# joey156/MECH5845M-WBC-for-Legged-Manipulator

Measured on AMD Instinct MI355X. Metric: wbc_qp_solves_per_sec, higher is better.
Workload: dtype f64

## Files before the change

mech5845m-wbc-for-legged-manipulator_amd/csrc/wbc_k_sim3p.hip:

```cpp
#include "wbc_packed.h"

namespace wbc {

#ifdef WBC_ABLATE
#define PSTOP(k, val) do { if (A.dbg_stop == 100 + (k)) { if (valid) { A.out.qdot[(size_t)b * NV + s] = (val); if (s == 0) A.out.status[b] = 0; } return; } } while (0)
#else
#define PSTOP(k, val) do { } while (0)
#endif
#ifdef SIM3P_NO_LAYOUT_HINTS
#define RARE(c) (c)
#else
#define RARE(c) __builtin_expect(!!(c), 0)
#endif
#define COLD_MARK() asm volatile("; WBC_COLD")
#ifndef SIM3P_WAVES
#define SIM3P_WAVES 2
#endif
template <bool WARM, bool TRUNK = false, bool QCON = false, bool ROT = false, bool TP = false, bool FIXD = false>
#ifdef SIM3P_NUM_VGPR
__attribute__((amdgpu_waves_per_eu(SIM3P_NUM_VGPR, SIM3P_NUM_VGPR)))
#endif
__global__ void __launch_bounds__(64, SIM3P_WAVES) wbc_tick_sim3p_kernel(const KernelArgs A, const DevModel* __restrict__ models,
                                                               const WbcConfig* __restrict__ cfgs, const DevPlan* __restrict__ plans,
                                                               const WbcTaskParams* __restrict__ tps, const WoGeom wg) {
#ifdef SIM3P_NUM_VGPR
  extern __shared__ double dyn_lds_[];
  union SUU { SmemP P; Smem G; };
  SUU& SU = *reinterpret_cast<SUU*>(dyn_lds_);
#else
  __shared__ union { SmemP P; Smem G; } SU;
#endif
  static_assert(sizeof(Smem) <= 20480 && sizeof(SmemP) <= 20480, "8 waves per CU");
  SmemP& SP = SU.P;
  const int lane = threadIdx.x, r = lane >> 4, s = lane & 15, rbase = lane & 48;
  PInst& I = SP.I[r];
  PVec& V = SP.V[r];
  const int grp = (int)blockIdx.x;
  const int pos = 4 * grp + r;
  const bool valid = pos < A.B;
  const int b = valid ? wo_instance(A.worder, wg, A.B, grp, r, pos) : A.B - 1;
  int mid = 0;
  if (A.in.model_id) { mid = A.in.model_id[b]; mid = mid < 0 ? 0 : (mid >= A.n_models ? A.n_models - 1 : mid); }
  const DevModel& M = models[mid];
  const WbcConfig& cfg = cfgs[mid];
  const DevPlan& P = plans[mid];
  const double dt = A.dt, inv_dt = 1.0 / A.dt;
  const WbcTaskParams* tpr = nullptr;
  bool tpbad = false;
  if (TP) {
    tpbad = tp_row_bad16(tps + b, s, rbase);
    tpr = tpbad ? reinterpret_cast<const WbcTaskParams*>(&cfg.ee_W[0][0]) : tps + b;
  }

  {
    const double* qg = A.in.q + (size_t)b * NQ;
    const double q0 = qg[s], q1 = (16 + s < NQ) ? qg[16 + s] : 0.0;
    double ex = 0.0;
    if (s < 3) ex = A.in.ee_target ? A.in.ee_target[(size_t)b * 15 + 12 + s] : 0.0;
    else if (s < 6) ex = A.in.prev_ee_target ? A.in.prev_ee_target[(size_t)b * 15 + 12 + (s - 3)] : 0.0;
    else if (s < 10) ex = A.in.trunk_box_center ? A.in.trunk_box_center[(size_t)b * 4 + (s - 6)] : 0.0;
    V.in[s] = q0;
    if (16 + s < 28) V.in[16 + s] = q1;
    if (s < 10) V.in[28 + s] = ex;
    V.cl[s] = 0.0; V.cl[16 + s] = 0.0;
    if (TRUNK) {
      static_assert(offsetof(PVec, tv) - offsetof(PVec, yv) == 16 * sizeof(double), "yv [14..15] runs on into tv");
      double* const tin = V.yv + 14;
      const double t0 = pk_trunk_input(A.in, b, s), t1 = (s < 2) ? pk_trunk_input(A.in, b, 16 + s) : 0.0;
      const double tw = (s < 13) ? (TP ? (&tpr->trunk_W[0])[s] : (&cfg.trunk_W[0])[s]) : 0.0;
      tin[s] = t0;
      if (s < 2) tin[16 + s] = t1;
      if (s < 13) V.xv[2 + s] = tw;
    }
    if (WARM && s < 2) {
      const unsigned long long w = (A.ws_in && valid) ? A.ws_in[2 * (size_t)b + s] : 0ull;
      V.in[38 + s] = __longlong_as_double((long long)w);
    }
    if (A.in.ee_ref_rot) {
      if (s < 9) { V.dv[s] = A.in.ee_ref_rot[(size_t)b * 45 + 36 + s]; V.yv[s] = A.in.ee_prev_rot[(size_t)b * 45 + 36 + s]; }
    }
  }
  double at6[6] = {0, 0, 0, 0, 0, 0};
  if (TRUNK) {
    WSYNC();
    const double* const qv = V.in;
    const double* tw = V.xv + 2;
    double Rt_[9], vel[6];
    pk_trunk_target_vel(qv, V.yv + 14, tw, I.M2, inv_dt, s, Rt_, vel);
    const double trunk_w = tw[6];
    double at[6] = {0, 0, 0, 0, 0, 0};
    {
      const int c = s < 3 ? s : (s < 6 ? s - 3 : 0);
      const double col[3] = {Rt_[c], Rt_[3 + c], Rt_[6 + c]};
      const double pr[3] = {qv[0], qv[1], qv[2]};
      double lin[3] = {col[0], col[1], col[2]}, ang[3] = {0, 0, 0};
      if (s >= 3) { ang[0] = col[0]; ang[1] = col[1]; ang[2] = col[2]; cross3(pr, ang, lin); }
#pragma unroll
      for (int rr = 0; rr < 3; ++rr) {
        at[rr] = (s < 6) ? (tw[rr] * lin[rr]) * trunk_w : 0.0;
        at[3 + rr] = (s < 6) ? (tw[3 + rr] * ang[rr]) * trunk_w : 0.0;
      }
    }
    double* const At2 = I.M1;
    WSYNC();
    if (s < 6) {
#pragma unroll
      for (int rr = 0; rr < 6; rr += 2) sts2(At2 + s * 6 + rr, at[rr], at[rr + 1]);
    }
    WSYNC();
#pragma unroll
    for (int rr = 0; rr < 6; ++rr) at6[rr] = at[rr];
    if (s < 6) {
      double vs = vel[0];
#pragma unroll
      for (int i = 1; i < 6; ++i) vs = (s == i) ? vel[i] : vs;
      V.pad_[s] = vs * trunk_w;
    }
    if (s < 6) {
      double gs = 0.0;
#pragma unroll
      for (int rr = 0; rr < 6; ++rr) gs = fma(-at[rr], vel[rr] * trunk_w, gs);
#pragma unroll
      for (int k = 0; k < 6; ++k) {
        const double2a t0 = lds2(At2 + k * 6), t1 = lds2(At2 + k * 6 + 2), t2 = lds2(At2 + k * 6 + 4);
        I.Cq[s * 6 + k] = fma(at[0], t0.x, fma(at[1], t0.y, fma(at[2], t1.x, fma(at[3], t1.y, fma(at[4], t2.x, at[5] * t2.y)))));
      }
      I.Cq[36 + s] = gs;
    }
    WSYNC();
    __builtin_amdgcn_sched_barrier(0);
  }
  const int nv = FIXD ? SIM3P_FIXD_NV : M.nv, nq = FIXD ? SIM3P_FIXD_NQ : M.nq, n = FIXD ? SIM3P_FIXD_N : P.n_red, nelim = FIXD ? SIM3P_FIXD_NELIM : P.nelim,
            nl = 3 * nelim, p_keep = FIXD ? SIM3P_FIXD_PKEEP : P.p_keep, p = p_keep + nl;
  const unsigned fl = P.flags;
  const bool c_con_trunk = fl & 2u;
  const int c_task_joint = (fl >> 4) & 7u;
  const bool has_grip = (P.task_ee_mask >> 4) & 1u;
  const DevPlan::PkCol cv = P.pk_var[s], cg = P.pk_leg[s];
  DevPlan::PkJoint fkn = P.pk_fk[0][s];
  const int scq0 = P.pk_scq[(2 + s) & 31], scq1 = P.pk_scq[(18 + s) & 31];
  const int dof0 = cv.dof, dof1 = cg.dof;
  const int c0_joint = cv.joint, c0_lin = cv.lin, c0_ang = cv.ang, c1_joint = cg.joint, c1_lin = cg.lin, c1_ang = cg.ang;
  const int dq0 = cv.dq_idx, dq1 = cg.dq_idx;
  const double dlo0 = cv.d_lo, dhi0 = cv.d_hi, dvm0 = cv.d_vm, dlo1 = cg.d_lo, dhi1 = cg.d_hi, dvm1 = cg.d_vm;
  const double dcoef = cfg.damper_coef, dqi = cfg.damper_qi, dqs = cfg.damper_qs;
  const int gj = M.frame_joint[WBC_FR_EE0 + 4];
  const double gp0 = M.frame_p[WBC_FR_EE0 + 4][0], gp1 = M.frame_p[WBC_FR_EE0 + 4][1], gp2 = M.frame_p[WBC_FR_EE0 + 4][2];
  const unsigned gsup = P.redsup[WBC_FR_EE0 + 4];
  const double ee_w = TPW(ee_w[4]);
  double eW[6], eG[3];
#pragma unroll
  for (int i = 0; i < 6; ++i) eW[i] = TPW(ee_W[4][i]);
#pragma unroll
  for (int i = 0; i < 3; ++i) eG[i] = TPW(ee_gain[4][i]);
  const double joint_w = TPW(joint_w), tb_z = cfg.trunk_box_z_frac, tb_a = cfg.trunk_box_ang, tb_s = cfg.trunk_box_scale;
  WSYNC();
  const double* const qv = V.in;
  PSTOP(6, qv[s] + dlo0 + dlo1 + eW[0] + (double)(fkn.joint + scq0 + scq1));
  double* const oMi = I.M1;
  double* const sc = I.M2 + PV * PLD - 48;
  pk_fk_seed(oMi, sc, qv, scq0, scq1, s);
  WSYNC();
  PSTOP(7, oMi[12 + s] + sc[4 + s]);
  pk_fk_sweep<ROT>(oMi, sc, qv, M, P.pk_fk, fkn, s);
  PSTOP(1, oMi[12 * 4 + (s & 7)]);
  double lin0[3] = {0, 0, 0}, ang0[3] = {0, 0, 0}, lin1[3] = {0, 0, 0};
  if (s < n) pk_jac_col(oMi, c0_joint, c0_lin, c0_ang, lin0, ang0);
  if (s < nl) { double a1[3]; pk_jac_col(oMi, c1_joint, c1_lin, c1_ang, lin1, a1); }
  double Rtr[9], ptr[3], pfe[3];
  {
    const double* Pr = oMi + 12 * M.frame_joint[WBC_FR_TRUNK];
#pragma unroll
    for (int c = 0; c < 3; ++c)
#pragma unroll
      for (int rr = 0; rr < 3; ++rr) Rtr[3 * rr + c] = Pr[3 * c + rr];
    ptr[0] = Pr[9]; ptr[1] = Pr[10]; ptr[2] = Pr[11];
    const double* Pg = oMi + 12 * gj;
#pragma unroll
    for (int rr = 0; rr < 3; ++rr) pfe[rr] = Pg[9 + rr] + Pg[rr] * gp0 + Pg[3 + rr] * gp1 + Pg[6 + rr] * gp2;
  }
  WSYNC();

  double* const At = I.M2;
  double* const Kb = I.M2 + 16 * 6;
  double* const Bb = I.M2 + 16 * 6 + 48;
  double g = 0.0;
  double a[6] = {0, 0, 0, 0, 0, 0};
  double bt[6] = {0, 0, 0, 0, 0, 0};
  if (has_grip) {
    const bool sup = (s < n) && ((gsup >> s) & 1u);
    double wxp[3];
    cross3(ang0, pfe, wxp);
#pragma unroll
    for (int rr = 0; rr < 3; ++rr) {
      a[rr] = sup ? eW[rr] * ((lin0[rr] + wxp[rr]) * ee_w) : 0.0;
      a[3 + rr] = sup ? eW[3 + rr] * (ang0[rr] * ee_w) : 0.0;
    }
    const double* xt = V.in + 28;
    const double* xp = V.in + 31;
#pragma unroll
    for (int i = 0; i < 3; ++i) {
      const double br = ((xt[i] - xp[i]) * inv_dt + eG[i] * ((xt[i] - pfe[i]) * inv_dt)) * ee_w;
      g = fma(-a[i], br, g);
      bt[i] = br;
    }
    if (A.in.ee_ref_rot) {
      const double* Rs = V.dv;
      const double* Rp = V.yv;
      double D[9];
#pragma unroll
      for (int i = 0; i < 9; ++i) D[i] = (Rs[i] - Rp[i]) * inv_dt;
      const double w3 = D[6] * Rs[3] + D[7] * Rs[4] + D[8] * Rs[5];
      const double w4 = D[0] * Rs[6] + D[1] * Rs[7] + D[2] * Rs[8];
      const double w5 = D[3] * Rs[0] + D[4] * Rs[1] + D[5] * Rs[2];
      g = fma(-a[3], w3 * ee_w, g); g = fma(-a[4], w4 * ee_w, g); g = fma(-a[5], w5 * ee_w, g);
      bt[3] = w3 * ee_w; bt[4] = w4 * ee_w; bt[5] = w5 * ee_w;
    }
  }
  if (TRUNK && s < 6) g += I.Cq[36 + s];
#pragma unroll
  for (int rr = 0; rr < 6; rr += 2) sts2(At + s * 6 + rr, a[rr], a[rr + 1]);
  if (!QCON) {
    if (s < nl) { Kb[4 * s] = lin1[0]; Kb[4 * s + 1] = lin1[1]; Kb[4 * s + 2] = lin1[2]; }
    if (s < 6) { Bb[4 * s] = lin0[0]; Bb[4 * s + 1] = lin0[1]; Bb[4 * s + 2] = lin0[2]; }
  }
  const double dpost = (1.0 / nv) * joint_w;
  double g1 = 0.0;
  double bp0 = 0.0, bp1 = 0.0;
  {
    const bool prev0 = (c_task_joint == WBC_JOINT_PREV) || (c_task_joint >= WBC_JOINT_MANI && !((P.post_zero >> dof0) & 1u));
    const bool prev1 = (c_task_joint == WBC_JOINT_PREV) || (c_task_joint >= WBC_JOINT_MANI && !((P.post_zero >> dof1) & 1u));
    double u0 = (prev0 && s < n) ? qv[dof0 < 6 ? dof0 : dof0 + 1] : 0.0;
    double u1 = (prev1 && s < nl) ? qv[dof1 < 6 ? dof1 : dof1 + 1] : 0.0;
    if (QCON && A.in.posture_u) {
      u0 = (s < n) ? A.in.posture_u[(size_t)b * NV + dof0] : 0.0;
      u1 = (s < nl) ? A.in.posture_u[(size_t)b * NV + dof1] : 0.0;
    }
    if (s < n) g = fma(-dpost, (1.0 / nv) * u0 * joint_w, g);
    if (s < nl) g1 = -dpost * ((1.0 / nv) * u1 * joint_w);
    bp0 = (s < n) ? (1.0 / nv) * u0 * joint_w : 0.0;
    bp1 = (s < nl) ? (1.0 / nv) * u1 * joint_w : 0.0;
  }
  if (s >= n) g = 0.0;
  if (RARE(A.post_static && P.post_pert)) {
    COLD_MARK();
    WSYNC();
    if (((P.post_pert >> s) & 1u)) V.in[s] = (qv[s] + 0.0002) - (0.0002 * 2);
    if (16 + s < NQ && ((P.post_pert >> (16 + s)) & 1u)) V.in[16 + s] = (qv[16 + s] + 0.0002) - (0.0002 * 2);
  }
  WSYNC();
  if (s < 6) {
    double v = bt[0];
#pragma unroll
    for (int i = 1; i < 6; ++i) v = (s == i) ? bt[i] : v;
    V.in[28 + s] = v;
  }
  double h[PV];
  {
#pragma unroll
    for (int k = 0; k < PV; ++k) {
      const double2a t0 = lds2(At + k * 6), t1 = lds2(At + k * 6 + 2), t2 = lds2(At + k * 6 + 4);
      h[k] = fma(a[0], t0.x, fma(a[1], t0.y, fma(a[2], t1.x, fma(a[3], t1.y, fma(a[4], t2.x, a[5] * t2.y)))));
    }
#pragma unroll
    for (int k = 0; k < PV; ++k) if (k == s) h[k] += (s < n) ? dpost * dpost : 1.0;
    if (TRUNK && s < 6) {
#pragma unroll
      for (int k = 0; k < 6; k += 2) { const double2a v = lds2(I.Cq + s * 6 + k); h[k] += v.x; h[k + 1] += v.y; }
    }
  }
  PSTOP(2, h[0] + h[5] + h[11] + g);
  if (QCON && A.in.q_con) {
    WSYNC();
    {
      const double* qg = A.in.q_con + (size_t)b * NQ;
      const double c0 = qg[s], c1 = (16 + s < NQ) ? qg[16 + s] : 0.0;
      V.in[s] = c0;
      if (16 + s < 28) V.in[16 + s] = c1;
    }
    fkn = P.pk_fk[0][s];
    WSYNC();
    pk_fk_seed(oMi, sc, qv, scq0, scq1, s);
    WSYNC();
#pragma unroll 1
    for (int L = 0; L < 5; ++L) {
      const DevPlan::PkJoint fk = fkn;
      if (L + 1 < 5) fkn = P.pk_fk[L + 1][s];
      const int j = fk.joint;
      if (j >= 0) {
        const bool rev = fk.rev != 0;
        const int a0 = fk.a0, a1 = fk.a1, a2 = fk.a2;
        const double* Pp = oMi + 12 * fk.parent;
        const double sn = rev ? sc[2 * j] : 0.0, cs = rev ? sc[2 * j + 1] : 1.0;
        const double pris = rev ? 0.0 : qv[fk.q_idx];
        if (ROT && fk.rot) {
          fk_place_rot_lds(oMi + 12 * j, Pp, M.rp[j], a0, a1, a2, sn, cs, pris);
        } else {
          double Av[3], Bv[3], Cv[3], Pv[3];
#pragma unroll
          for (int rr = 0; rr < 3; ++rr) { Av[rr] = Pp[a0 + rr]; Bv[rr] = Pp[a1 + rr]; Cv[rr] = Pp[a2 + rr]; Pv[rr] = Pp[9 + rr]; }
          double* Po = oMi + 12 * j;
// ... 589 lines not shown
      if (stepping && ++iters > max_iter) { status = WBC_QP_MAX_ITER; stepping = false; searching = false; }
      if (RARE(__ballot(stepping && drop_l >= 0) != 0)) {
        const bool dr = stepping && drop_l >= 0;
        drop_slot(dr, drop_l);
        V.xv[s] = x;
        WSYNC();
        if (dr) {
          double v;
          if (is_row) {
            const double2a c0 = lds2(I.Cq + rr_ * 6), c1 = lds2(I.Cq + rr_ * 6 + 2), c2 = lds2(I.Cq + rr_ * 6 + 4);
            const double2a x0 = lds2(V.xv), x1 = lds2(V.xv + 2), x2 = lds2(V.xv + 4);
            v = fma(c0.x, x0.x, fma(c0.y, x0.y, fma(c1.x, x1.x, fma(c1.y, x1.y, fma(c2.x, x2.x, c2.y * x2.y)))));
          } else v = V.xv[ip & 15];
          s_ip = sgn * v - b_ip;
          drop_l = -1;
        }
      }
      if (!__ballot(stepping)) break;
      double d = normal_d(is_row, rr_, ip, sgn);
      if (!has_b || !stepping) d = 0.0;
      WSYNC();
      V.dv[s] = d; V.yv[s] = (s >= q) ? d : 0.0;
      WSYNC();
      const double zn = rsum16a(s >= q ? d * d : 0.0);
      const Zr zr = products(__ballot(stepping && q > 0) != 0);
      const double z = zr.z, rv = zr.rv;
      const bool have_step = zn > 100.0 * n * EPS2 * jf2 * np2;
      const bool cand = (s < q) && (rv > 2.2250738585072014e-308);
      const double ratio = cand ? u * frcp(rv) : INFINITY;
      const double t1 = rmin16a(ratio);
      const unsigned long long lm = __ballot(cand && ratio == t1);
      const int l = (t1 < INFINITY) ? __ffs((int)((lm >> rbase) & 0xFFFFull)) - 1 : -1;
      const double t2 = have_step ? -s_ip * frcp(zn) : INFINITY;
      const double t = fmin(t1, t2);
      if (stepping && !(t < INFINITY)) { status = WBC_QP_INFEASIBLE; stepping = false; searching = false; }
      if (stepping) {
        if (have_step) x = fma(t, z, x);
        u = fma(-t, rv, u);
        u_ip += t;
      }
      const bool add = stepping && have_step && t == t2;
      if (__ballot(add)) {
        add_step(add, zn, zr, wc, is_row, rr_, ip, u_ip);
        if (add) stepping = false;
      }
      if (stepping) drop_l = l;
    }
  }
#ifndef SIM3P_LATE_ATOMIC
  const int wocls = wo_class(iters, flagged);
  WoPost wop = {0ull, 0ull, 0u, 0u, (uint32_t)WO_NS + 1u, 0u};
  if (A.worder) wop = wo_post(A.worder, wg, grp, valid, wocls, r, s);
#endif
#ifdef WBC_ABLATE
  const bool skip_refine_ = A.dbg_stop == 109;
#else
  const bool skip_refine_ = false;
#endif
  if (A.refine > 0 && !skip_refine_) {
    WSYNC();
    V.xv[s] = has_b ? x : 0.0;
    V.yv[s] = 0.0;
    if (WARM) { V.cl[s] = lb; V.cl[16 + s] = ub; V.tv[s] = clb; V.dv[s] = cub; }
    WSYNC();
    const double2a x0 = lds2(V.xv), x1_ = lds2(V.xv + 2), x2 = lds2(V.xv + 4);
    auto rowval = [&](const int rr_) -> double {
      const double2a c0 = lds2(I.Cq + rr_ * 6), c1 = lds2(I.Cq + rr_ * 6 + 2), c2 = lds2(I.Cq + rr_ * 6 + 4);
      return fma(c0.x, x0.x, fma(c0.y, x0.y, fma(c1.x, x1_.x, fma(c1.y, x1_.y, fma(c2.x, x2.x, c2.y * x2.y)))));
    };
    const double vrow = has_r ? rowval(s) : 0.0;
    const int cc = a_code & 255, sd = (a_code >> 8) & 1;
    const bool slot = s < q, srow = slot && cc >= n;
    const int rr_ = srow ? ((cc - n) & 15) : 0, iv = cc & 15;
    const double sgn = sd ? -1.0 : 1.0;
    const double us = slot ? sgn * u : 0.0;
    double r2 = 0.0;
    if (WARM) {
      const double vbd = V.xv[iv];
      const double val = srow ? rowval(rr_) : vbd;
      const double* const bsrc = srow ? ((sd ? V.dv : V.tv) + rr_) : (V.cl + (sd ? 16 : 0) + iv);
      r2 = slot ? sgn * (*bsrc - val) : 0.0;
    }
    const double bpl = bperm(bp1, rbase + ((s - p_keep) & 15));
    const double wl = (s >= p_keep && s < p) ? dpost * (bpl - dpost * vrow) : 0.0;
    WSYNC();
    V.xv[s] = wl;
    if (srow) V.yv[rr_] = us;
    if (slot && !srow) V.dv[iv] = us;
    if (WARM) V.cl[s] = r2;
    double r1 = 0.0;
    {
      const double2a b0 = lds2(V.in + 28), b1 = lds2(V.in + 30), b2 = lds2(V.in + 32);
      const double btv[6] = {b0.x, b0.y, b1.x, b1.y, b2.x, b2.y};
      const double xm = has_b ? x : 0.0;
#pragma unroll
      for (int rr = 0; rr < 6; ++rr) {
        double pr = a[rr] * xm;
        asm volatile("" : "+v"(pr));
        r1 = fma(a[rr], btv[rr] - rsum16a(pr), r1);
      }
      if (TRUNK) {
        const double2a t0 = lds2(V.pad_), t1 = lds2(V.pad_ + 2), t2 = lds2(V.pad_ + 4);
        const double ttv[6] = {t0.x, t0.y, t1.x, t1.y, t2.x, t2.y};
#pragma unroll
        for (int rr = 0; rr < 6; ++rr) {
          double pr = at6[rr] * xm;
// ... 21 lines not shown
#pragma unroll
    for (int j = 0; j < PV; j += 2) {
      const double2a r1v = lds2(V.tv + j);
      dy2 = fma(J[j * PLD + sv], r1v.x, fma(J[(j + 1) * PLD + sv], r1v.y, dy2));
      if (WARM) {
        const double2a r2v = lds2(V.cl + j);
        dy1 = fma(T[j * PLD + sv], r2v.x, fma(T[(j + 1) * PLD + sv], r2v.y, dy1));
      }
    }
    V.yv[s] = (s < PV) ? ((s < q) ? dy1 : dy2) : 0.0;
    WSYNC();
    double da = 0.0, db = 0.0;
#pragma unroll
    for (int k = 0; k < PV; k += 2) { const double2a j2 = lds2(J + sv * PLD + k), w2 = lds2(V.yv + k); da = fma(j2.x, w2.x, da); db = fma(j2.y, w2.y, db); }
    const double dxl = has_b ? da + db : 0.0;
    const double dmax = -rmin16a(-fabs(dxl)), xmax = fmax(1.0, -rmin16a(has_b ? -fabs(x) : 0.0));
    const bool nanr = ((__ballot(dxl != dxl) >> rbase) & 0xFFFFull) != 0;
    if (has_b && status == WBC_QP_OPTIMAL && !nanr && dmax <= 0.25 * xmax) x += dxl;
  }
  if (status == WBC_QP_OPTIMAL) {
    const unsigned long long bad = __ballot(has_b && !(fabs(x) <= 1.7976931348623157e308));
    if ((bad >> rbase) & 0xFFFFull) status = WBC_QP_NUMERICAL;
  }
  if (TP && tpbad) status = WBC_QP_NUMERICAL;
  if (status != WBC_QP_OPTIMAL) x = 0.0;
  if (WARM && A.ws_out) {
    const int cc = a_code & 255, sd = (a_code >> 8) & 1;
    const int dA = bpermi(dofA, rbase + (cc & 15));
    const int dR = bpermi(dofR, rbase + ((cc - n) & 15));
    unsigned long long w0 = 0ull, w1 = 0ull;
    if (status == WBC_QP_OPTIMAL && s < q) {
      if (cc < n) w0 = 1ull << (32 * sd + (dA & 31));
      else if (cc - n < p_keep) w1 = 1ull << (32 * sd + ((cc - n) & 31));
      else w0 = 1ull << (32 * sd + (dR & 31));
    }
    w0 = ror16a(w0); w1 = ror16a(w1);
    if (valid && !flagged && s == 0) { A.ws_out[2 * (size_t)b] = w0; A.ws_out[2 * (size_t)b + 1] = w1; }
  }

  WSYNC();
  V.xv[s] = has_b ? x : 0.0;
  V.cl[s] = 0.0; V.cl[16 + s] = 0.0;
  WSYNC();
  double x1 = 0.0;
  if (s < nl) {
    const double2a v0 = lds2(V.xv), v1 = lds2(V.xv + 2), v2 = lds2(V.xv + 4);
    const double2a g0 = lds2(I.Cq + (p_keep + s) * 6), g1_ = lds2(I.Cq + (p_keep + s) * 6 + 2), g2 = lds2(I.Cq + (p_keep + s) * 6 + 4);
    x1 = fma(g0.x, v0.x, fma(g0.y, v0.y, fma(g1_.x, v1.x, fma(g1_.y, v1.y, fma(g2.x, v2.x, g2.y * v2.y)))));
    V.cl[dofB] = x1;
  }
  if (s < n) V.cl[dofA] = x;
  WSYNC();
  const bool wr = valid && !flagged;
  if (wr) {
    double* qo = A.out.qdot + (size_t)b * NV;
    qo[s] = V.cl[s];
    if (16 + s < NV) qo[16 + s] = V.cl[16 + s];
    if (s == 0) {
      A.out.status[b] = status;
      if (A.out.iters) A.out.iters[b] = iters + nl + P.nlock;
    }
  }
  if (A.out.q_next) {
    WSYNC();
    V.xv[s] = (s < 6) ? V.cl[s] * dt : 0.0;
    WSYNC();
    double* qn = A.out.q_next + (size_t)b * NQ;
    if (wr) {
      integrate_ff(V, s, qn);
#pragma unroll
      for (int hh = 0; hh < 2; ++hh) {
        const int d = 6 + s + 16 * hh;
        if (d < nv) { const int qi = M.col_q[d]; qn[qi] = qv[qi] + V.cl[d] * dt; }
      }
      if (s < NQ - nq) qn[nq + s] = 0.0;
    }
  }
  if (A.worder) {
#ifdef SIM3P_LATE_ATOMIC
    const int wocls = wo_class(iters, flagged);
    const WoPost wop = wo_post(A.worder, wg, grp, valid, wocls, r, s);
#endif
    wo_finish(A.worder, wg, A.B, valid, b, wocls, r, s, wop);
  }
#ifndef WBC_NO_TAIL
  const unsigned long long tailm = __ballot(valid && flagged && s == 0);
  if (RARE(tailm != 0)) {
    asm volatile("; WBC_TAIL_BEGIN" ::: "memory");
#pragma unroll 1
    for (int rr = 0; rr < 4; ++rr) {
      if (!((tailm >> (16 * rr)) & 1ull)) continue;
      tail_instance<WARM, false, ROT, TP>(&SU.G, __builtin_amdgcn_readlane(b, 16 * rr), models, cfgs, plans);
    }
  }
#endif
}

#ifndef SIM3P_PART
#define SIM3P_PART -1
#endif
#define WBC_PART SIM3P_PART
#define WBC_KERNEL wbc_tick_sim3p_kernel
#define WBC_KPARAMS (const KernelArgs, const DevModel* __restrict__, const WbcConfig* __restrict__, const DevPlan* __restrict__, const WbcTaskParams* __restrict__, const WoGeom)
typedef void (*Sim3pKernel) WBC_KPARAMS;
#define SIM3P_VARIANTS(V)  \
  V(0, false, false, false, false, false) \
  V(1, true, false, false, false, false)  \
  V(1, false, true, false, false, false)  \
  V(1, true, true, false, false, false)   \
  V(2, false, false, true, false, false)  \
  V(2, true, false, true, false, false)   \
  V(3, false, false, false, true, false)  \
  V(3, true, false, false, true, false)   \
  V(3, false, true, false, true, false)   \
  V(3, true, true, false, true, false)    \
  V(4, false, false, true, true, false)   \
  V(4, true, false, true, true, false)    \
  V(5, false, false, false, false, true)  \
  V(5, true, false, false, false, true)   \
  V(5, false, true, false, false, true)   \
  V(6, true, true, false, false, true)    \
  V(6, false, false, true, false, true)   \
  V(6, true, false, true, false, true)    \
  V(7, false, false, false, true, true)   \
  V(7, true, false, false, true, true)    \
  V(7, false, true, false, true, true)    \
// ... 60 lines not shown
```

mech5845m-wbc-for-legged-manipulator_amd/csrc/wbc_packed.h:

```cpp
#pragma once
#include "wbc_common.h"
#include "wbc_wave_geom.h"

namespace wbc {

constexpr int PLD = 14;
constexpr int PN = 16;
constexpr int PV = 12;
struct __attribute__((aligned(16))) PInst {
  double M1[PV * PLD];
  double M2[PV * PLD];
  double Cq[PN * 6];
  double pad_[8];
};
struct __attribute__((aligned(16))) PVec {
  double in[40];
  double xv[PN], dv[PN], yv[PN], tv[PN];
  double cl[32];
  double pad_[8];
};
static_assert(sizeof(PInst) % 256 == 192, "matrix blocks: 192 B (mod the 256-byte bank row) apart");
static_assert(sizeof(PVec) % 256 == 128, "vector blocks: half a bank row apart (mod 256 B)");
struct __attribute__((aligned(16))) SmemP { PInst I[4]; PVec V[4]; };

// ... 225 lines not shown
  double tx = T[srow * LDT + l];
  double jx = J[sJ * LDJ + l];
  double hrun = T[l * LDT + l];
  const int kend = dr ? q - 1 : 0;
#pragma unroll 1
  for (int k0 = 0; k0 < NT - 1; ++k0) {
    const bool on = dr && (l + k0 < kend);
    if (!__ballot(on)) break;
    const int k = on ? l + k0 : 0;
    const PkGivens g = pk_givens(hrun, T[l * LDT + k + 1]);
    const double ty_ = T[srow * LDT + k + 1];
    const double jy = J[sJ * LDJ + k + 1];
    WSYNC();
    if (on) {
      hrun = g.rho;
      if (s < q - 1) T[s * LDT + k] = fma(g.c, tx, g.s * ty_);
      if (has_b) J[s * LDJ + k] = fma(g.c, jx, g.s * jy);
      tx = fma(-g.s, tx, g.c * ty_);
      jx = fma(-g.s, jx, g.c * jy);
    }
    WSYNC();
  }
  WSYNC();
  if (dr) {
    if (s < q) T[s * LDT + q - 1] = 0.0;
  }
  WSYNC();
  if (dr) {
    if (s < q) T[(q - 1) * LDT + s] = 0.0;
    if (has_b) J[s * LDJ + q - 1] = jx;
    --q;
  }
  WSYNC();
}

__device__ __forceinline__ int wo_class(const int iters, const bool tail) {
  return (tail || iters >= 10) ? 0 : iters >= 6 ? 1 : iters >= 3 ? 2 : 5 - iters;
}
__device__ __forceinline__ uint32_t* wo_list(WaveOrder* wo, const uint32_t l, const int g, const int c) {
  return reinterpret_cast<uint32_t*>(wo + WO_NS) + ((size_t)(l * WO_NS + g) * WO_NCLS + c) * WO_CAP;
}
static_assert(WO_GEOM_SW == (uint32_t)WO_SW && WO_GEOM_XMAX > (uint32_t)(WO_SW * WO_NS), "wbc_wave_geom.h: the slice width; the reciprocal's range covers every grid the order takes");
__device__ __forceinline__ uint32_t wo_divk(const WoGeom& wg, const uint32_t x) {
#ifdef SIM3P_WO_DIVIDE
  return (uint32_t)((int)x / (int)wg.ns);
#else
  return wo_div(wg, x);
#endif
}
__device__ __forceinline__ int wo_instance(WaveOrder* __restrict__ wo, const WoGeom& wg, const int B, const int grp, const int r, const int pos) {
  if (!wo || wg.ns > (uint32_t)WO_NS) return pos;
  const uint32_t k = wo_divk(wg, (uint32_t)grp), g = wo_mod(wg, (uint32_t)grp, k);
  const WaveOrder& sl = wo[g];
  if (sl.B != (uint32_t)B) return pos;
  const uint32_t cur = sl.cur & 1u, j = 4u * k + (uint32_t)r;
  uint32_t d = 0;
#pragma unroll
  for (int c = 1; c < WO_NCLS; ++c) {
    const uint32_t o = sl.off[c];
    if (j >= o) d = (uint32_t)(c * WO_CAP) - o;
  }
  const uint32_t i = wo_list(wo, cur, g, 0)[min(j + d, (uint32_t)(WO_NCLS * WO_CAP) - 1u)];
  return i < (uint32_t)B ? (int)i : B - 1;
}
struct WoPost { unsigned long long old, add; unsigned same; uint32_t cur, ns, g; };
__device__ __forceinline__ WoPost wo_post(WaveOrder* wo, const WoGeom& wg, const int grp, const bool valid, const int cls, const int r, const int s) {
  WoPost t; t.old = 0ull; t.add = 1ull << 54; t.same = 0u; t.cur = 0u;
  t.ns = wg.ns; t.g = 0u;
  if (t.ns > (uint32_t)WO_NS) return t;
  t.g = wo_mod(wg, (uint32_t)grp, wo_divk(wg, (uint32_t)grp));
  t.cur = wo[t.g].cur & 1u;
  const unsigned long long vm = __ballot(valid && s == 0);
#pragma unroll
  for (int k = 0; k < 4; ++k) {
    const int ck = __builtin_amdgcn_readlane(cls, 16 * k);
    const bool vk = (vm >> (16 * k)) & 1ull;
    t.same |= (vk && ck == cls) ? 1u << k : 0u;
    t.add += vk ? 1ull << (9 * ck) : 0ull;
  }
  if (r == 0 && s == 0) {
#ifdef SIM3P_LATE_ATOMIC
    t.old = atomicAdd(&wo[t.g].word[t.cur ^ 1u], t.add);
#else
    uint32_t wi = t.cur ^ 1u;
    asm volatile("" : "+v"(wi));
    t.old = atomicAdd(&wo[t.g].word[wi & 1u], t.add);
#endif
  }
  return t;
}
__device__ __forceinline__ void wo_finish(WaveOrder* wo, const WoGeom& wg, const int B, const bool valid, const int b, const int cls, const int r,
                                          const int s, const WoPost& t) {
  const uint32_t ns = t.ns, g = t.g;
  if (ns > (uint32_t)WO_NS) return;
  WaveOrder& sl = wo[g];
  const uint32_t cur = t.cur, nxt = cur ^ 1u;
  const unsigned long long old =
      ((unsigned long long)(uint32_t)__builtin_amdgcn_readfirstlane((int)(t.old >> 32)) << 32) | (uint32_t)__builtin_amdgcn_readfirstlane((int)t.old);
  const uint32_t at = (uint32_t)((old >> (9 * cls)) & 511ull) + (uint32_t)__popc(t.same & ((1u << r) - 1u));
  if (valid && s == 0 && at < WO_CAP) wo_list(wo, nxt, g, cls)[at] = (uint32_t)b;
#ifdef SIM3P_WO_DIVIDE
  const int G_ = (int)gridDim.x;
  const uint32_t nwaves = (uint32_t)((G_ - (int)g + (int)ns - 1) / (int)ns);
#else
  const uint32_t nwaves = wg.wq + (g < wg.wr ? 1u : 0u);
#endif
  if (r == 0 && s == 0 && (uint32_t)(old >> 54) == nwaves - 1u) {
    const unsigned long long fin = old + t.add;
    uint32_t n = 0u;
#pragma unroll
    for (int c = 0; c < WO_NCLS; ++c) { sl.off[c] = n; n += (uint32_t)((fin >> (9 * c)) & 511ull); }
    const uint32_t G = gridDim.x, glast = (wg.wr ? wg.wr : ns) - 1u;
    const uint32_t expect = 4u * nwaves - ((g == glast) ? 4u * G - (uint32_t)B : 0u);
    sl.B = (n == expect) ? (uint32_t)B : 0u;
// ... 21 lines not shown
    quat_to_R(qv + 3, Rt);
#pragma unroll
    for (int c = 0; c < 3; ++c)
#pragma unroll
      for (int rr = 0; rr < 3; ++rr) oMi[12 + 3 * c + rr] = Rt[3 * rr + c];
    oMi[12 + 9] = qv[0]; oMi[12 + 10] = qv[1]; oMi[12 + 11] = qv[2];
  }
}
template <bool ROT, int NLEV>
__device__ __forceinline__ void pk_fk_sweep(double* const oMi, const double* const sc, const double* const qv, const DevModel& M,
                                            const DevPlan::PkJoint (&sched)[NLEV][16], DevPlan::PkJoint& fkn, const int s) {
#pragma unroll 1
  for (int L = 0; L < NLEV; ++L) {
    const DevPlan::PkJoint fk = fkn;
    if (L + 1 < NLEV) fkn = sched[L + 1][s];
    const int j = fk.joint;
    if (j >= 0) {
      const bool rev = fk.rev != 0;
      const int a0 = fk.a0, a1 = fk.a1, a2 = fk.a2;
      const double* Pp = oMi + 12 * fk.parent;
      const double sn = rev ? sc[2 * j] : 0.0, cs = rev ? sc[2 * j + 1] : 1.0;
      const double pris = rev ? 0.0 : qv[fk.q_idx];
      if (ROT && fk.rot) {
        fk_place_rot_lds(oMi + 12 * j, Pp, M.rp[j], a0, a1, a2, sn, cs, pris);
      } else {
        double Av[3], Bv[3], Cv[3], Pv[3];
#pragma unroll
        for (int rr = 0; rr < 3; ++rr) { Av[rr] = Pp[a0 + rr]; Bv[rr] = Pp[a1 + rr]; Cv[rr] = Pp[a2 + rr]; Pv[rr] = Pp[9 + rr]; }
        double* Po = oMi + 12 * j;
#pragma unroll
        for (int rr = 0; rr < 3; ++rr) {
          Po[a0 + rr] = Av[rr];
          Po[a1 + rr] = cs * Bv[rr] + sn * Cv[rr];
          Po[a2 + rr] = cs * Cv[rr] - sn * Bv[rr];
          Po[9 + rr] = Pv[rr] + Av[rr] * (fk.t0 + pris) + Bv[rr] * fk.t1 + Cv[rr] * fk.t2;
        }
      }
    }
    WSYNC();
  }
}
__device__ __forceinline__ void pk_jac_col(const double* const oMi, const int joint, const int lin_axis, const int ang_axis, double (&lin)[3],
                                           double (&ang)[3]) {
  const double* Pj = oMi + 12 * joint;
  const double pj[3] = {Pj[9], Pj[10], Pj[11]};
  if (ang_axis >= 0) { ang[0] = Pj[3 * ang_axis]; ang[1] = Pj[3 * ang_axis + 1]; ang[2] = Pj[3 * ang_axis + 2]; cross3(pj, ang, lin); }
  if (lin_axis >= 0) { lin[0] = Pj[3 * lin_axis]; lin[1] = Pj[3 * lin_axis + 1]; lin[2] = Pj[3 * lin_axis + 2]; }
}

__device__ __forceinline__ double pk_trunk_input(const WbcTickIn& in, const int b, const int k) {
  return (k < 3) ? in.trunk_target[(size_t)b * 3 + k] : (k < 6) ? in.prev_trunk_target[(size_t)b * 3 + (k - 3)]
       : (k < 9) ? in.trunk_ref_euler[(size_t)b * 3 + (k - 6)] : in.trunk_prev_rot[(size_t)b * 9 + (k - 9)];
}
__device__ __forceinline__ double pk_ee_omega(const WbcTickIn& in, const int b, const int s, const double inv_dt) {
  double om = 0.0;
  if (in.ee_ref_rot && s < 15) {
    const int e = s / 3, i = s - 3 * e;
    const double* Rs = in.ee_ref_rot + (size_t)b * 45 + 9 * e;
    const double* Rp = in.ee_prev_rot + (size_t)b * 45 + 9 * e;
    const int ra = (i == 0) ? 6 : ((i == 1) ? 0 : 3), rb = (i == 0) ? 3 : ((i == 1) ? 6 : 0);
    om = ((Rs[ra] - Rp[ra]) * inv_dt) * Rs[rb] + ((Rs[ra + 1] - Rp[ra + 1]) * inv_dt) * Rs[rb + 1] + ((Rs[ra + 2] - Rp[ra + 2]) * inv_dt) * Rs[rb + 2];
  }
  return om;
}
template <bool TP>
__device__ __forceinline__ bool pk_stage_weights(double* const wt, const WbcConfig& cfg, const WbcTaskParams* const tps, const int b, const int s,
                                                 const int rbase, const int ncfg) {
  const double* cw = &cfg.ee_W[0][0];
  bool tpbad = false;
  if (TP) {
    const double* rw = reinterpret_cast<const double*>(tps + b);
    bool bad = false;
#pragma unroll
    for (int i = 0; i < 6; ++i) {
      const int k = s + 16 * i;
      const double v = (k < WBC_TASK_PARAMS_DOUBLES) ? rw[k] : ((k < ncfg) ? cw[k] : 0.0);
      bad = bad || (k < WBC_TASK_PARAMS_DOUBLES && tp_entry_bad(k, v));
      wt[s + 16 * i] = v;
    }
    tpbad = ((__ballot(bad) >> rbase) & 0xFFFFull) != 0ull;
  }
  if (!TP || tpbad) {
#pragma unroll
    for (int i = 0; i < 6; ++i) wt[s + 16 * i] = (s + 16 * i < ncfg) ? cw[s + 16 * i] : 0.0;
  }
  return tpbad;
}
__device__ __forceinline__ void pk_trunk_target_vel(const double* const qv, const double* const tin, const double* const tw, double* const sh,
                                                    const double inv_dt, const int s, double (&Rt_)[9], double (&vel)[6]) {
  const double* xt = tin;
  const double* xp = tin + 3;
  const double* er = tin + 6;
  double fq[4], rq[4], Rs[9];
  quat_to_R(qv + 3, Rt_);
  R_to_quat(Rt_, fq);
  {
    const SinCos t = sincos_cw(s < 3 ? er[s < 3 ? s : 0] : 0.5 * er[(s < 6 ? s : 3) - 3]);
    if (s < 6) { sh[2 * s] = t.s; sh[2 * s + 1] = t.c; }
    WSYNC();
    const double sa = sh[0], ca = sh[1], sb = sh[2], cb = sh[3], sc_ = sh[4], cc = sh[5];
    euler_to_R(sa, ca, sb, cb, sc_, cc, Rs);
    const double qx[4] = {sh[6], 0, 0, sh[7]}, qy[4] = {0, sh[8], 0, sh[9]}, qz[4] = {0, 0, sh[10], sh[11]};
    double tq[4];
    quat_mul(qy, qx, tq);
    quat_mul(qz, tq, rq);
  }
// ... 15 lines not shown
```

Baseline: 456.3 million.

## Batch kernel-entry global loads and hoist per-model table reads before dependent work

Restructures the kernel prologue so the per-instance input loads (q, ee targets, rotations, warm start, trunk inputs, model id) are all issued together before a scheduling barrier, instead of serially after the model-id lookup. Per-model plan and config fields are gathered into one table struct, and some late reads (trunk frame joint, post_zero/post_pert, nlock, col_q) are hoisted early and pinned with asm barriers so they are not re-loaded near the end. The wave-order slice header is read as eight scalar words at once. This aims to overlap global-memory latency at kernel entry and exit, at the cost of higher register pressure and more complex code.

```diff
diff --git a/mech5845m-wbc-for-legged-manipulator_amd/csrc/wbc_entry_in.h b/mech5845m-wbc-for-legged-manipulator_amd/csrc/wbc_entry_in.h
--- /dev/null
+++ b/mech5845m-wbc-for-legged-manipulator_amd/csrc/wbc_entry_in.h
@@ -0,0 +1,37 @@
+#pragma once
+#include <stdint.h>
+
+#if defined(__HIPCC__) || defined(__CUDACC__)
+#define WBC_ENTRY_FN __host__ __device__ __forceinline__
+#else
+#define WBC_ENTRY_FN static inline
+#endif
+
+namespace wbc {
+
+enum : int { EIN_EE_TARGET = 0, EIN_PREV_EE_TARGET = 1, EIN_TRUNK_BOX_CENTER = 2, EIN_EE_REF_ROT = 3, EIN_COUNT = 4 };
+constexpr int EIN_ROW[EIN_COUNT] = {15, 15, 4, 45};
+
+struct EntryIn {
+  int arr;
+  int64_t off;
+  bool on;
+};
+
+WBC_ENTRY_FN EntryIn entry_in_ex(const int s, const int64_t b, const unsigned present) {
+  EntryIn e;
+  e.arr = s < 3 ? EIN_EE_TARGET : (s < 6 ? EIN_PREV_EE_TARGET : EIN_TRUNK_BOX_CENTER);
+  const int row = s < 6 ? 15 : 4, col = s < 3 ? 12 + s : (s < 6 ? 12 + (s - 3) : s - 6);
+  e.off = b * row + col;
+  e.on = s < 10 && ((present >> e.arr) & 1u);
+  return e;
+}
+WBC_ENTRY_FN EntryIn entry_in_rot(const int s, const int64_t b, const unsigned present) {
+  EntryIn e;
+  e.arr = EIN_EE_REF_ROT;
+  e.off = b * 45 + 36 + s;
+  e.on = s < 9 && ((present >> EIN_EE_REF_ROT) & 1u);
+  return e;
+}
+
+}
diff --git a/mech5845m-wbc-for-legged-manipulator_amd/csrc/wbc_k_sim3p.hip b/mech5845m-wbc-for-legged-manipulator_amd/csrc/wbc_k_sim3p.hip
--- a/mech5845m-wbc-for-legged-manipulator_amd/csrc/wbc_k_sim3p.hip
+++ b/mech5845m-wbc-for-legged-manipulator_amd/csrc/wbc_k_sim3p.hip
@@ -1,4 +1,5 @@
 #include "wbc_packed.h"
+#include "wbc_entry_in.h"
 
 namespace wbc {
 
@@ -16,6 +17,46 @@
 #ifndef SIM3P_WAVES
 #define SIM3P_WAVES 2
 #endif
+template <bool TP, bool FIXD>
+struct PkTab {
+  DevPlan::PkCol cv, cg;
+  DevPlan::PkJoint fkn;
+  int scq0, scq1, gj, tj, nv, nq, n_red, nelim, p_keep;
+  unsigned flags, task_ee_mask, gsup, post_zero, post_pert;
+  double dcoef, dqi, dqs, gp[3], tb_z, tb_a, tb_s, ee_w, eW[6], eG[3], joint_w;
+};
+template <bool TP, bool FIXD>
+__device__ __forceinline__ PkTab<TP, FIXD> pk_tab_load(const DevModel& M, const WbcConfig& cfg, const DevPlan& P, const int s) {
+  PkTab<TP, FIXD> t;
+  t.cv = P.pk_var[s]; t.cg = P.pk_leg[s];
+  t.fkn = P.pk_fk[0][s];
+  t.scq0 = P.pk_scq[(2 + s) & 31]; t.scq1 = P.pk_scq[(18 + s) & 31];
+  t.gj = M.frame_joint[WBC_FR_EE0 + 4];
+#ifdef SIM3P_ENTRY_OLD_LATE
+  t.tj = 0;
+#else
+  t.tj = M.frame_joint[WBC_FR_TRUNK];
+#endif
+  t.nv = FIXD ? SIM3P_FIXD_NV : M.nv; t.nq = FIXD ? SIM3P_FIXD_NQ : M.nq; t.n_red = FIXD ? SIM3P_FIXD_N : P.n_red;
+  t.nelim = FIXD ? SIM3P_FIXD_NELIM : P.nelim; t.p_keep = FIXD ? SIM3P_FIXD_PKEEP : P.p_keep;
+  t.flags = P.flags; t.task_ee_mask = P.task_ee_mask; t.gsup = P.redsup[WBC_FR_EE0 + 4];
+#ifdef SIM3P_ENTRY_OLD_LATE
+  t.post_zero = t.post_pert = 0u;
+#else
+  t.post_zero = P.post_zero; t.post_pert = P.post_pert;
+#endif
+  t.dcoef = cfg.damper_coef; t.dqi = cfg.damper_qi; t.dqs = cfg.damper_qs;
+#pragma unroll
+  for (int i = 0; i < 3; ++i) t.gp[i] = M.frame_p[WBC_FR_EE0 + 4][i];
+  t.tb_z = cfg.trunk_box_z_frac; t.tb_a = cfg.trunk_box_ang; t.tb_s = cfg.trunk_box_scale;
+  t.ee_w = TP ? 0.0 : (double)cfg.ee_w[4];
+#pragma unroll
+  for (int i = 0; i < 6; ++i) t.eW[i] = TP ? 0.0 : (double)cfg.ee_W[4][i];
+#pragma unroll
+  for (int i = 0; i < 3; ++i) t.eG[i] = TP ? 0.0 : (double)cfg.ee_gain[4][i];
+  t.joint_w = TP ? 0.0 : (double)cfg.joint_w;
+  return t;
+}
 template <bool WARM, bool TRUNK = false, bool QCON = false, bool ROT = false, bool TP = false, bool FIXD = false>
 #ifdef SIM3P_NUM_VGPR
 __attribute__((amdgpu_waves_per_eu(SIM3P_NUM_VGPR, SIM3P_NUM_VGPR)))
@@ -38,15 +79,70 @@
   const int grp = (int)blockIdx.x;
   const int pos = 4 * grp + r;
   const bool valid = pos < A.B;
+  const bool mid_known = FIXD || !A.in.model_id;
+  int mid = 0;
+  asm("" : "+v"(mid));
+#ifdef SIM3P_ENTRY_OLD_SLICE
   const int b = valid ? wo_instance(A.worder, wg, A.B, grp, r, pos) : A.B - 1;
-  int mid = 0;
+#else
+  const int bw = wo_instance(A.worder, wg, A.B, grp, r, pos);
+  const int b = valid ? bw : A.B - 1;
+#endif
+  const double dt = A.dt, inv_dt = 1.0 / A.dt;
+  const WbcTaskParams* tpr = nullptr;
+  bool tpbad = false;
+#ifndef SIM3P_ENTRY_OLD_INPUTS
+  double tw = 0.0;
+  bool tw_late = TRUNK;
+  {
+    const double* qg = A.in.q + (size_t)b * NQ;
+    const unsigned present = (A.in.ee_target ? 1u << EIN_EE_TARGET : 0u) | (A.in.prev_ee_target ? 1u << EIN_PREV_EE_TARGET : 0u) |
+                             (A.in.trunk_box_center ? 1u << EIN_TRUNK_BOX_CENTER : 0u) | (A.in.ee_ref_rot ? 1u << EIN_EE_REF_ROT : 0u);
+    const EntryIn ie = entry_in_ex(s, b, present), ir = entry_in_rot(s, b, present);
+    const double* const eb = ie.arr == EIN_EE_TARGET ? A.in.ee_target : (ie.arr == EIN_PREV_EE_TARGET ? A.in.prev_ee_target : A.in.trunk_box_center);
+    const double q0 = qg[s];
+    double q1 = 0.0, ex = 0.0, rs = 0.0, rp = 0.0, t0 = 0.0, t1 = 0.0;
+    unsigned long long wsw = 0ull;
+    int midv = 0;
+    if (16 + s < NQ) q1 = qg[16 + s];
+    if (ie.on) ex = eb[ie.off];
+    if (ir.on) { rs = A.in.ee_ref_rot[ir.off]; rp = A.in.ee_prev_rot[ir.off]; }
+    if (WARM && s < 2 && A.ws_in && valid) wsw = A.ws_in[2 * (size_t)b + s];
+    if (!FIXD && A.in.model_id) midv = A.in.model_id[b];
+    if (TRUNK) {
+      t0 = *pk_trunk_input_at(A.in, b, s);
+      if (s < 2) t1 = *pk_trunk_input_at(A.in, b, 16 + s);
+      if (!TP && mid_known) { tw_late = false; if (s < 13) tw = (&cfgs[mid].trunk_W[0])[s]; }
+    }
+    __builtin_amdgcn_sched_barrier(0);
+    if (!FIXD && A.in.model_id) mid = midv < 0 ? 0 : (midv >= A.n_models ? A.n_models - 1 : midv);
+    if (TP) {
+      tpbad = tp_row_bad16(tps + b, s, rbase);
+      tpr = tpbad ? reinterpret_cast<const WbcTaskParams*>(&cfgs[mid].ee_W[0][0]) : tps + b;
+    }
+    V.in[s] = q0;
+    if (16 + s < 28) V.in[16 + s] = q1;
+    if (s < 10) V.in[28 + s] = ex;
+    V.cl[s] = 0.0; V.cl[16 + s] = 0.0;
+    if (TRUNK) {
+      static_assert(offsetof(PVec, tv) - offsetof(PVec, yv) == 16 * sizeof(double), "yv [14..15] runs on into tv");
+      double* const tin = V.yv + 14;
+      if (tw_late && s < 13) tw = TP ? (&tpr->trunk_W[0])[s] : (&cfgs[mid].trunk_W[0])[s];
+      tin[s] = t0;
+      if (s < 2) tin[16 + s] = t1;
+      if (s < 13) V.xv[2 + s] = tw;
+    }
+    if (WARM && s < 2) V.in[38 + s] = __longlong_as_double((long long)wsw);
+    if (ir.on) { V.dv[s] = rs; V.yv[s] = rp; }
+  }
+  const DevModel& M = models[mid];
+  const WbcConfig& cfg = cfgs[mid];
+  const DevPlan& P = plans[mid];
+#else
   if (A.in.model_id) { mid = A.in.model_id[b]; mid = mid < 0 ? 0 : (mid >= A.n_models ? A.n_models - 1 : mid); }
   const DevModel& M = models[mid];
   const WbcConfig& cfg = cfgs[mid];
   const DevPlan& P = plans[mid];
-  const double dt = A.dt, inv_dt = 1.0 / A.dt;
-  const WbcTaskParams* tpr = nullptr;
-  bool tpbad = false;
   if (TP) {
     tpbad = tp_row_bad16(tps + b, s, rbase);
     tpr = tpbad ? reinterpret_cast<const WbcTaskParams*>(&cfg.ee_W[0][0]) : tps + b;
@@ -80,6 +176,7 @@
       if (s < 9) { V.dv[s] = A.in.ee_ref_rot[(size_t)b * 45 + 36 + s]; V.yv[s] = A.in.ee_prev_rot[(size_t)b * 45 + 36 + s]; }
     }
   }
+#endif
   double at6[6] = {0, 0, 0, 0, 0, 0};
   if (TRUNK) {
     WSYNC();
@@ -130,30 +227,31 @@
     WSYNC();
     __builtin_amdgcn_sched_barrier(0);
   }
-  const int nv = FIXD ? SIM3P_FIXD_NV : M.nv, nq = FIXD ? SIM3P_FIXD_NQ : M.nq, n = FIXD ? SIM3P_FIXD_N : P.n_red, nelim = FIXD ? SIM3P_FIXD_NELIM : P.nelim,
-            nl = 3 * nelim, p_keep = FIXD ? SIM3P_FIXD_PKEEP : P.p_keep, p = p_keep + nl;
-  const unsigned fl = P.flags;
+  const PkTab<TP, FIXD> tab = pk_tab_load<TP, FIXD>(M, cfg, P, s);
+  const int nv = FIXD ? SIM3P_FIXD_NV : tab.nv, nq = FIXD ? SIM3P_FIXD_NQ : tab.nq, n = FIXD ? SIM3P_FIXD_N : tab.n_red, nelim = FIXD ? SIM3P_FIXD_NELIM : tab.nelim,
+            nl = 3 * nelim, p_keep = FIXD ? SIM3P_FIXD_PKEEP : tab.p_keep, p = p_keep + nl;
+  const unsigned fl = tab.flags;
   const bool c_con_trunk = fl & 2u;
   const int c_task_joint = (fl >> 4) & 7u;
-  const bool has_grip = (P.task_ee_mask >> 4) & 1u;
-  const DevPlan::PkCol cv = P.pk_var[s], cg = P.pk_leg[s];
-  DevPlan::PkJoint fkn = P.pk_fk[0][s];
-  const int scq0 = P.pk_scq[(2 + s) & 31], scq1 = P.pk_scq[(18 + s) & 31];
+  const bool has_grip = (tab.task_ee_mask >> 4) & 1u;
+  const DevPlan::PkCol cv = tab.cv, cg = tab.cg;
+  DevPlan::PkJoint fkn = tab.fkn;
+  const int scq0 = tab.scq0, scq1 = tab.scq1;
   const int dof0 = cv.dof, dof1 = cg.dof;
   const int c0_joint = cv.joint, c0_lin = cv.lin, c0_ang = cv.ang, c1_joint = cg.joint, c1_lin = cg.lin, c1_ang = cg.ang;
   const int dq0 = cv.dq_idx, dq1 = cg.dq_idx;
   const double dlo0 = cv.d_lo, dhi0 = cv.d_hi, dvm0 = cv.d_vm, dlo1 = cg.d_lo, dhi1 = cg.d_hi, dvm1 = cg.d_vm;
-  const double dcoef = cfg.damper_coef, dqi = cfg.damper_qi, dqs = cfg.damper_qs;
-  const int gj = M.frame_joint[WBC_FR_EE0 + 4];
-  const double gp0 = M.frame_p[WBC_FR_EE0 + 4][0], gp1 = M.frame_p[WBC_FR_EE0 + 4][1], gp2 = M.frame_p[WBC_FR_EE0 + 4][2];
-  const unsigned gsup = P.redsup[WBC_FR_EE0 + 4];
-  const double ee_w = TPW(ee_w[4]);
+  const double dcoef = tab.dcoef, dqi = tab.dqi, dqs = tab.dqs;
+  const int gj = tab.gj;
+  const double gp0 = tab.gp[0], gp1 = tab.gp[1], gp2 = tab.gp[2];
+  const unsigned gsup = tab.gsup;
+  const double ee_w = TP ? (double)tpr->ee_w[4] : tab.ee_w;
   double eW[6], eG[3];
 #pragma unroll
-  for (int i = 0; i < 6; ++i) eW[i] = TPW(ee_W[4][i]);
-#pragma unroll
-  for (int i = 0; i < 3; ++i) eG[i] = TPW(ee_gain[4][i]);
-  const double joint_w = TPW(joint_w), tb_z = cfg.trunk_box_z_frac, tb_a = cfg.trunk_box_ang, tb_s = cfg.trunk_box_scale;
+  for (int i = 0; i < 6; ++i) eW[i] = TP ? (double)tpr->ee_W[4][i] : tab.eW[i];
+#pragma unroll
+  for (int i = 0; i < 3; ++i) eG[i] = TP ? (double)tpr->ee_gain[4][i] : tab.eG[i];
+  const double joint_w = TP ? (double)tpr->joint_w : tab.joint_w, tb_z = tab.tb_z, tb_a = tab.tb_a, tb_s = tab.tb_s;
   WSYNC();
   const double* const qv = V.in;
   PSTOP(6, qv[s] + dlo0 + dlo1 + eW[0] + (double)(fkn.joint + scq0 + scq1));
@@ -169,7 +267,11 @@
   if (s < nl) { double a1[3]; pk_jac_col(oMi, c1_joint, c1_lin, c1_ang, lin1, a1); }
   double Rtr[9], ptr[3], pfe[3];
   {
+#ifdef SIM3P_ENTRY_OLD_LATE
     const double* Pr = oMi + 12 * M.frame_joint[WBC_FR_TRUNK];
+#else
+    const double* Pr = oMi + 12 * tab.tj;
+#endif
 #pragma unroll
     for (int c = 0; c < 3; ++c)
 #pragma unroll
@@ -228,8 +330,13 @@
   double g1 = 0.0;
   double bp0 = 0.0, bp1 = 0.0;
   {
-    const bool prev0 = (c_task_joint == WBC_JOINT_PREV) || (c_task_joint >= WBC_JOINT_MANI && !((P.post_zero >> dof0) & 1u));
-    const bool prev1 = (c_task_joint == WBC_JOINT_PREV) || (c_task_joint >= WBC_JOINT_MANI && !((P.post_zero >> dof1) & 1u));
+#ifdef SIM3P_ENTRY_OLD_LATE
+    const unsigned post_zero = P.post_zero;
+#else
+    const unsigned post_zero = tab.post_zero;
+#endif
+    const bool prev0 = (c_task_joint == WBC_JOINT_PREV) || (c_task_joint >= WBC_JOINT_MANI && !((post_zero >> dof0) & 1u));
+    const bool prev1 = (c_task_joint == WBC_JOINT_PREV) || (c_task_joint >= WBC_JOINT_MANI && !((post_zero >> dof1) & 1u));
     double u0 = (prev0 && s < n) ? qv[dof0 < 6 ? dof0 : dof0 + 1] : 0.0;
     double u1 = (prev1 && s < nl) ? qv[dof1 < 6 ? dof1 : dof1 + 1] : 0.0;
     if (QCON && A.in.posture_u) {
@@ -242,11 +349,16 @@
     bp1 = (s < nl) ? (1.0 / nv) * u1 * joint_w : 0.0;
   }
   if (s >= n) g = 0.0;
-  if (RARE(A.post_static && P.post_pert)) {
+#ifdef SIM3P_ENTRY_OLD_LATE
+  const unsigned post_pert = P.post_pert;
+#else
+  const unsigned post_pert = tab.post_pert;
+#endif
+  if (RARE(A.post_static && post_pert)) {
     COLD_MARK();
     WSYNC();
-    if (((P.post_pert >> s) & 1u)) V.in[s] = (qv[s] + 0.0002) - (0.0002 * 2);
-    if (16 + s < NQ && ((P.post_pert >> (16 + s)) & 1u)) V.in[16 + s] = (qv[16 + s] + 0.0002) - (0.0002 * 2);
+    if (((post_pert >> s) & 1u)) V.in[s] = (qv[s] + 0.0002) - (0.0002 * 2);
+    if (16 + s < NQ && ((post_pert >> (16 + s)) & 1u)) V.in[16 + s] = (qv[16 + s] + 0.0002) - (0.0002 * 2);
   }
   WSYNC();
   if (s < 6) {
@@ -942,6 +1054,13 @@
   WoPost wop = {0ull, 0ull, 0u, 0u, (uint32_t)WO_NS + 1u, 0u};
   if (A.worder) wop = wo_post(A.worder, wg, grp, valid, wocls, r, s);
 #endif
+#ifndef SIM3P_ENTRY_OLD_LATE
+  int nlock = P.nlock, cq0 = 0, cq1 = 0;
+  if (A.out.q_next) {
+    if (6 + s < nv) cq0 = M.col_q[6 + s];
+    if (22 + s < nv) cq1 = M.col_q[22 + s];
+  }
+#endif
 #ifdef WBC_ABLATE
   const bool skip_refine_ = A.dbg_stop == 109;
 #else
@@ -1069,13 +1188,18 @@
   if (s < n) V.cl[dofA] = x;
   WSYNC();
   const bool wr = valid && !flagged;
+#ifdef SIM3P_ENTRY_OLD_LATE
+  const int nlock = P.nlock;
+#else
+  asm volatile("" : "+v"(nlock));
+#endif
   if (wr) {
     double* qo = A.out.qdot + (size_t)b * NV;
     qo[s] = V.cl[s];
     if (16 + s < NV) qo[16 + s] = V.cl[16 + s];
     if (s == 0) {
       A.out.status[b] = status;
-      if (A.out.iters) A.out.iters[b] = iters + nl + P.nlock;
+      if (A.out.iters) A.out.iters[b] = iters + nl + nlock;
     }
   }
   if (A.out.q_next) {
@@ -1083,12 +1207,19 @@
     V.xv[s] = (s < 6) ? V.cl[s] * dt : 0.0;
     WSYNC();
     double* qn = A.out.q_next + (size_t)b * NQ;
+#ifndef SIM3P_ENTRY_OLD_LATE
+    asm volatile("" : "+v"(cq0), "+v"(cq1));
+#endif
     if (wr) {
       integrate_ff(V, s, qn);
 #pragma unroll
       for (int hh = 0; hh < 2; ++hh) {
         const int d = 6 + s + 16 * hh;
+#ifdef SIM3P_ENTRY_OLD_LATE
         if (d < nv) { const int qi = M.col_q[d]; qn[qi] = qv[qi] + V.cl[d] * dt; }
+#else
+        if (d < nv) { const int qi = hh ? cq1 : cq0; qn[qi] = qv[qi] + V.cl[d] * dt; }
+#endif
       }
       if (s < NQ - nq) qn[nq + s] = 0.0;
     }
diff --git a/mech5845m-wbc-for-legged-manipulator_amd/csrc/wbc_packed.h b/mech5845m-wbc-for-legged-manipulator_amd/csrc/wbc_packed.h
--- a/mech5845m-wbc-for-legged-manipulator_amd/csrc/wbc_packed.h
+++ b/mech5845m-wbc-for-legged-manipulator_amd/csrc/wbc_packed.h
@@ -301,6 +301,7 @@
   if (!wo || wg.ns > (uint32_t)WO_NS) return pos;
   const uint32_t k = wo_divk(wg, (uint32_t)grp), g = wo_mod(wg, (uint32_t)grp, k);
   const WaveOrder& sl = wo[g];
+#ifdef SIM3P_ENTRY_OLD_SLICE
   if (sl.B != (uint32_t)B) return pos;
   const uint32_t cur = sl.cur & 1u, j = 4u * k + (uint32_t)r;
   uint32_t d = 0;
@@ -309,6 +310,22 @@
     const uint32_t o = sl.off[c];
     if (j >= o) d = (uint32_t)(c * WO_CAP) - o;
   }
+#else
+  static_assert(offsetof(WaveOrder, cur) == 16 && offsetof(WaveOrder, B) == 20 && offsetof(WaveOrder, off) == 24, "cur, B, off[0..5]: eight words from byte 16");
+  uint32_t w[8];
+  const uint32_t* const wp = reinterpret_cast<const uint32_t*>(&sl) + 4;
+#pragma unroll
+  for (int i = 0; i < 8; ++i) w[i] = wp[i];
+  asm volatile("" : "+s"(w[0]), "+s"(w[1]), "+s"(w[2]), "+s"(w[3]), "+s"(w[4]), "+s"(w[5]), "+s"(w[6]), "+s"(w[7]));
+  if (w[1] != (uint32_t)B) return pos;
+  const uint32_t cur = w[0] & 1u, j = 4u * k + (uint32_t)r;
+  uint32_t d = 0;
+#pragma unroll
+  for (int c = 1; c < WO_NCLS; ++c) {
+    const uint32_t o = w[2 + c];
+    if (j >= o) d = (uint32_t)(c * WO_CAP) - o;
+  }
+#endif
   const uint32_t i = wo_list(wo, cur, g, 0)[min(j + d, (uint32_t)(WO_NCLS * WO_CAP) - 1u)];
   return i < (uint32_t)B ? (int)i : B - 1;
 }
@@ -436,6 +453,11 @@
   return (k < 3) ? in.trunk_target[(size_t)b * 3 + k] : (k < 6) ? in.prev_trunk_target[(size_t)b * 3 + (k - 3)]
        : (k < 9) ? in.trunk_ref_euler[(size_t)b * 3 + (k - 6)] : in.trunk_prev_rot[(size_t)b * 9 + (k - 9)];
 }
+__device__ __forceinline__ const double* pk_trunk_input_at(const WbcTickIn& in, const int b, const int k) {
+  const double* const base = (k < 3) ? in.trunk_target : (k < 6) ? in.prev_trunk_target : (k < 9) ? in.trunk_ref_euler : in.trunk_prev_rot;
+  const size_t off = (k < 3) ? (size_t)b * 3 + k : (k < 6) ? (size_t)b * 3 + (k - 3) : (k < 9) ? (size_t)b * 3 + (k - 6) : (size_t)b * 9 + (k - 9);
+  return base + off;
+}
 __device__ __forceinline__ double pk_ee_omega(const WbcTickIn& in, const int b, const int s, const double inv_dt) {
   double om = 0.0;
   if (in.ee_ref_rot && s < 15) {
```

After: 474.3 million, median of 6. +3.9%, better.
